# lifuguan/GGRt_official

Measured on AMD Instinct MI355X. Metric: Gaussian raster fwd+bwd Mpix/s @1M Gaussians 1080p, higher is better.
Workload: dtype f32; 1 GPU; C3: 1000000 Gaussians, 1920x1080, SH deg 3, profile A, fwd+bwd incl. camera gradient, 1 frame per GPU; parallelism=frames x1

## Files before the change

ggrt_official_amd/csrc/api.hip:

```cpp
#include "../../include/ggr_raster.h"
#include "ggr_common.h"
#include "blend_feat.h"
#include "blend_contrib.h"
#include "blend_pick.h"
#include "blend_dist.h"
#include <algorithm>
#include <mutex>
#include <vector>

#include <stdarg.h>
#include <stdio.h>
#include <stdlib.h>
#include <string.h>
#include <time.h>

namespace {

thread_local char g_err[512] = "";
const char kSpinFault[] = "depth sort: a look-back spin hit its bound (GPU preempted or halted?); frame not rendered";
const char kRangeFault[] = "depth sort: a sort key beyond 30 bits reached the sort (keys must come from preprocess_fwd); frame not rendered";

int fail(int code, const char* fmt, ...) {
    va_list ap;
    va_start(ap, fmt);
// ... 665 lines not shown
        uint32_t two[2] = {0u, 0u};
        HIP_TRY(hipMemcpyAsync(two, g.counters, 8, hipMemcpyDeviceToHost, s));
        HIP_TRY(hipStreamSynchronize(s));
        if (two[1] & 2u) return fail(GGR_E_HIP, "%s", kSpinFault);
        if (two[1] & 4u) return fail(GGR_E_LIMIT, "%s", kRangeFault);
    }
    if (bucket_slow && out->depth_sort_used == GGR_DEPTH_SORT_GLOBAL) out->depth_sort_used = GGR_DEPTH_SORT_GLOBAL_SLOW;
    tm.finish();
    if (out->stage_ms && side) {
        float ms = 0.f;
        if (hipEventElapsedTime(&ms, side->t0, side->t1) == hipSuccess) out->stage_ms[GGR_FWD_COLOUR] += ms;
        else (void)hipGetLastError();
    }
    return GGR_OK;
}

int backward_impl(const GgrSettings* st, const ViewSet& vs, const GgrBackwardIn* in, GgrBackwardOut* out, void* stream,
                  const float* dL_dalpha) {
    if (!out) return fail(GGR_E_INVALID, "null gradient output struct");
    const int NV = vs.V;
    if (st->num_points == 0) {
        hipStream_t s0 = (hipStream_t)stream;
        if (out->dL_dviewmatrix) HIP_TRY(hipMemsetAsync(out->dL_dviewmatrix, 0, 64 * (size_t)NV, s0));
        if (out->dL_dprojmatrix) HIP_TRY(hipMemsetAsync(out->dL_dprojmatrix, 0, 64 * (size_t)NV, s0));
        if (out->dL_dcampos) HIP_TRY(hipMemsetAsync(out->dL_dcampos, 0, 12 * (size_t)NV, s0));
        return GGR_OK;
    }
    if (!out->dL_dmeans3D || !out->dL_dmeans2D || !out->dL_dopacities || !out->dL_dcov3D)
        return fail(GGR_E_INVALID, "null gradient output");
    if (!in->geom_buffer || !in->image_buffer || !in->scratch || !in->dL_dout_color)
        return fail(GGR_E_INVALID, "null saved buffer / scratch / upstream gradient");
    const bool has_cp = in->fwd.colors_precomp != nullptr;
    if (has_cp ? !out->dL_dcolors_precomp : !out->dL_dshs) return fail(GGR_E_INVALID, "null colour gradient output");
    const bool has_sr = in->fwd.scales != nullptr;
    if (has_sr && (!out->dL_dscales || !out->dL_drotations)) return fail(GGR_E_INVALID, "null scale/rotation gradient output");
    if (in->fwd.aux_precomp && in->dL_dout_depth && !out->dL_daux) return fail(GGR_E_INVALID, "null dL_daux output");
    const int npose = (out->dL_dviewmatrix != nullptr) + (out->dL_dprojmatrix != nullptr) + (out->dL_dcampos != nullptr);
    if (npose != 0 && npose != 3) return fail(GGR_E_INVALID, "camera gradients: give all three outputs or none");
    hipStream_t s = (hipStream_t)stream;
    const int P = st->num_points, W = st->image_width, H = st->image_height;
    const bool dbg = st->debug != 0;
    if (in->num_rendered != 0 && !in->binning_buffer) return fail(GGR_E_INVALID, "null binning buffer");

    GeomLayout g = ggr_carve_geom((void*)in->geom_buffer, (size_t)P * NV, ggr_sort_segments((size_t)NV));
    ImageLayout im = ggr_carve_image((void*)in->image_buffer, W, H, NV);
    const uint32_t* point_list = (const uint32_t*)in->binning_buffer;
    BwdScratch sc = ggr_carve_bwd(in->scratch, (size_t)P, (size_t)NV);

    StageTimer tm(s, out->stage_ms, GGR_BWD_STAGES);
    if (!in->scratch_zeroed)
        HIP_TRY(hipMemsetAsync(in->scratch, 0, sc.bytes, s));
    tm.mark(GGR_BWD_CLEAR);

    if (in->num_rendered != 0) {
        ggr::launch_blend_bwd(W, H, im.ranges, point_list, g.splat, g.colour, vs.bg, im.final_T, im.n_contrib,
                              in->dL_dout_color, in->dL_dout_depth, dL_dalpha, sc.grad2d, im.tile_top, im.ckpt,
                              im.ckpt_slots, im.bwd_segments, NV, s);
        KCHECK(dbg, s, "blend_bwd");
    }
    tm.mark(GGR_BWD_BLEND);
    const float* cov = in->fwd.cov3D_precomp ? in->fwd.cov3D_precomp : g.cov3D;
    ggr::launch_preprocess_bwd(P, st->sh_degree, st->sh_stride, in->fwd.means3D, in->fwd.shs, g.sh_jac, has_cp ? 1 : 0,
                               in->fwd.scales, in->fwd.rotations, st->scale_modifier, cov, vs, W, H, in->radii, g.clamped,
                               sc.grad2d, in->dL_dout_depth ? 1 : 0, out->dL_dmeans3D, out->dL_dmeans2D,
                               out->dL_dopacities, out->dL_dshs, out->dL_dcolors_precomp, out->dL_dcov3D,
                               out->dL_dscales, out->dL_drotations, in->fwd.aux_precomp ? out->dL_daux : nullptr,
                               npose ? sc.pose_acc : nullptr, out->dL_dviewmatrix, out->dL_dprojmatrix,
                               out->dL_dcampos, input_form(st, &in->fwd, vs.sets, out->dL_dshs), in->fwd.cov3D_precomp ? 1 : 0,
                               in->fwd.opacities, g.counters + GGR_CTR_ANTIALIAS , s);
    KCHECK(dbg, s, "preprocess_bwd");
    tm.mark(GGR_BWD_PREPROCESS);
    return GGR_OK;
}

}

extern "C" {

int ggr_forward_ext(const GgrSettings* st, const GgrForwardOptions* opt, const GgrForwardExtra* ex, const GgrForwardIn* in,
                    GgrForwardOut* out, GgrAllocFn alloc, void* alloc_ctx, void* stream) {
    g_err[0] = 0;
    int aa = 0;
    int rc = validate_options(opt, &aa);
    if (rc) return rc;
    if ((rc = validate_extra(ex, "GgrForwardExtra")) != 0) return rc;
    rc = validate(st, in);
    if (rc) return rc;
    return forward_impl(st, single_view(st, in), in, out, alloc, alloc_ctx, stream, aa, ex ? ex->out_alpha : nullptr);
}

int ggr_forward_opt(const GgrSettings* st, const GgrForwardOptions* opt, const GgrForwardIn* in, GgrForwardOut* out,
                    GgrAllocFn alloc, void* alloc_ctx, void* stream) {
    return ggr_forward_ext(st, opt, nullptr, in, out, alloc, alloc_ctx, stream);
}

int ggr_forward(const GgrSettings* st, const GgrForwardIn* in, GgrForwardOut* out, GgrAllocFn alloc,
                void* alloc_ctx, void* stream) {
    return ggr_forward_ext(st, nullptr, nullptr, in, out, alloc, alloc_ctx, stream);
}

int ggr_backward_ext(const GgrSettings* st, const GgrBackwardExtra* ex, const GgrBackwardIn* in, GgrBackwardOut* out,
                     void* stream) {
    g_err[0] = 0;
    int rc = validate_extra(ex, "GgrBackwardExtra");
    if (rc) return rc;
    if (!in) return fail(GGR_E_INVALID, "null inputs");
    rc = validate(st, &in->fwd);
    if (rc) return rc;
    return backward_impl(st, single_view(st, &in->fwd), in, out, stream, ex ? ex->dL_dout_alpha : nullptr);
}
// ... 430 lines not shown
```

ggrt_official_amd/csrc/blend_bwd.hip:

```cpp
#include "blend_common.h"

namespace ggr {

#define BATCH GGR_BATCH
#define RB 8

__device__ unsigned long long g_bwd_counters[4];
void blend_bwd_counters(unsigned long long* out, int reset) {
    (void)hipMemcpyFromSymbol(out, HIP_SYMBOL(g_bwd_counters), sizeof(g_bwd_counters));
    if (reset) { const unsigned long long z[4] = {0, 0, 0, 0}; (void)hipMemcpyToSymbol(HIP_SYMBOL(g_bwd_counters), z, sizeof z); }
}

template <int CTRL>
__device__ __forceinline__ float dpp_mov(float v) {
    return __int_as_float(__builtin_amdgcn_update_dpp(__float_as_int(v), __float_as_int(v), CTRL, 0xf, 0xf, true));
}

__device__ __forceinline__ float transpose_rows8(float (&v)[RB], int lane) {
    float w4[4];
    const bool h32 = (lane & 32) != 0;
#pragma unroll
    for (int i = 0; i < 4; i++) {
        const float keep = h32 ? v[i + 4] : v[i], send = h32 ? v[i] : v[i + 4];
        w4[i] = keep + __int_as_float(__builtin_amdgcn_ds_bpermute((lane ^ 32) << 2, __float_as_int(send)));
    }
    float w2[2];
#pragma unroll
    for (int i = 0; i < 2; i++) {
        const auto r = __builtin_amdgcn_permlane16_swap(__float_as_uint(w4[i]), __float_as_uint(w4[i + 2]), false, false);
        w2[i] = __uint_as_float(r[0]) + __uint_as_float(r[1]);
    }
    const bool hi = (lane & 8) != 0;
    const float keep = hi ? w2[1] : w2[0];
    const float send = hi ? w2[0] : w2[1];
    return keep + dpp_mov<0x128>(send);
}

__device__ __forceinline__ float sum_cols8(float s) {
    s += dpp_mov<0xB1>(s);
    s += dpp_mov<0x4E>(s);
    s += dpp_mov<0x141>(s);
    asm volatile("" : "+v"(s));
    return s;
}

__device__ __forceinline__ float transpose_cols8(const float (&o)[8], int lane) {
    const bool up = (lane & 4) != 0;
    const bool e0 = (((lane ^ (lane >> 2)) & 1) != 0), e1 = ((((lane >> 1) ^ (lane >> 2)) & 1) != 0);
    float k1[4], k2[2];
#pragma unroll
    for (int i = 0; i < 4; i++) {
        const float keep = e0 ? o[2 * i + 1] : o[2 * i], send = e0 ? o[2 * i] : o[2 * i + 1];
        k1[i] = keep + dpp_mov<0xB1>(send);
    }
#pragma unroll
    for (int j = 0; j < 2; j++) {
        const float keep = e1 ? k1[2 * j + 1] : k1[2 * j], send = e1 ? k1[2 * j] : k1[2 * j + 1];
        k2[j] = keep + dpp_mov<0x4E>(send);
    }
    const float keep = up ? k2[1] : k2[0], send = up ? k2[0] : k2[1];
    return keep + dpp_mov<0x141>(send);
}

template <bool HAS_DEPTH, bool HAS_ALPHA>
__global__ void __launch_bounds__(256)
blend_bwd_kernel(int W, int H, int grid_x, const uint2* __restrict__ ranges,
                 const uint32_t* __restrict__ point_list, const float4* __restrict__ splat,
                 const float4* __restrict__ colour,
                 const float* __restrict__ bg, const float* __restrict__ final_T,
                 const uint32_t* __restrict__ n_contrib, const float* __restrict__ dL_dpix,
                 const float* __restrict__ dL_ddepth, const float* __restrict__ dL_dalpha, float* __restrict__ grad2d,
                 const uint32_t* __restrict__ tile_top, const float* __restrict__ ckpt, int ckpt_slots,
                 int segments, int views) {
    __shared__ StagedSplat stage[BATCH];
    __shared__ __attribute__((aligned(16))) uint16_t surv[4][BATCH];
    __shared__ uint32_t wave_top[4];

    const int tid = threadIdx.x, lane = tid & 63, wave = tid >> 6;
    const int tiles1 = grid_x * ((H + GGR_TILE - 1) / GGR_TILE), ntiles = tiles1 * views;
    const int seg = segments > 1 ? (int)blockIdx.x / xcd_grid(ntiles) : 0;
    const int vtile = xcd_tile((int)blockIdx.x - seg * xcd_grid(ntiles), ntiles, true);
    if (vtile < 0) return;
    const int view = vtile / tiles1, tile = vtile - view * tiles1;
    const int tile_x = tile % grid_x, tile_y = tile / grid_x;
    const int qx0 = tile_x * GGR_TILE + (wave & 1) * 8, qy0 = tile_y * GGR_TILE + (wave >> 1) * 8;
    const int px = qx0 + (lane & 7), py = qy0 + (lane >> 3);
    const bool inside = px < W && py < H;
    const float pixx = (float)px, pixy = (float)py;
    const float rx0 = (float)qx0, ry0 = (float)qy0;
    const float qcx = rx0 + 3.5f, qcy = ry0 + 3.5f;
    const float pxc = (float)(lane & 7) - 3.5f, pyc = (float)(lane >> 3) - 3.5f;
    const float rx1 = (float)min(qx0 + 7, W - 1), ry1 = (float)min(qy0 + 7, H - 1);

    const uint2 range = ranges[vtile];
    const int top = (int)min(tile_top[vtile], range.y - range.x);
    int seg_lo = 0, seg_hi = top, stride = 0;
    if (segments > 1) {
        stride = ckpt_stride((int)(range.y - range.x), ckpt_slots, ntiles);
        seg_lo = seg * stride;
        seg_hi = min(top, seg_lo + stride);
    }
    if (seg_lo >= seg_hi) return;
    const size_t hw = (size_t)H * W;
    const size_t pid = inside ? (size_t)py * W + px : 0;
    {
        const size_t vo = (size_t)view * hw;
        final_T += vo; n_contrib += vo; dL_dpix += 3 * vo; bg += 3 * view;
        if (HAS_DEPTH) dL_ddepth += vo;
        if (HAS_ALPHA) dL_dalpha += vo;
        if (ckpt) ckpt += (size_t)ckpt_slots * GGR_CKPT_FLOATS * vo;
    }

    const float T_final = inside ? final_T[pid] : 0.f;
    uint32_t last = inside ? n_contrib[pid] : 0u;
    float dp0 = 0.f, dp1 = 0.f, dp2 = 0.f, dpz = 0.f, dpa = 0.f;
    if (inside) {
        dp0 = dL_dpix[pid]; dp1 = dL_dpix[hw + pid]; dp2 = dL_dpix[2 * hw + pid];
        if (HAS_DEPTH) dpz = dL_ddepth[pid];
        if (HAS_ALPHA) dpa = dL_dalpha[pid];
    }
    if (dp0 == 0.f && dp1 == 0.f && dp2 == 0.f && dpz == 0.f && (!HAS_ALPHA || dpa == 0.f)) last = 0u;
    const float bg_dot = bg[0] * dp0 + bg[1] * dp1 + bg[2] * dp2;
    const float ddelx_dx = 0.5f * (float)W, ddely_dy = 0.5f * (float)H;

    uint32_t wl = last;
#pragma unroll
    for (int off = 32; off > 0; off >>= 1) wl = max(wl, (uint32_t)__shfl_xor((int)wl, off));
    if (lane == 0) wave_top[wave] = wl;
    __syncthreads();
    seg_hi = min(seg_hi, (int)max(max(wave_top[0], wave_top[1]), max(wave_top[2], wave_top[3])));
    if (seg_lo >= seg_hi) return;

    float T = T_final;
    float R = T_final * (HAS_ALPHA ? bg_dot - dpa : bg_dot);
    float amax = GGR_ALPHA_MAX, amin = GGR_ALPHA_MIN;
    __asm__ volatile("" : "+s"(amax), "+s"(amin));

    if (stride > 0 && seg_hi == seg_lo + stride && last > (uint32_t)seg_hi) {
        const float* ck = ckpt + (size_t)(seg_hi / stride) * GGR_CKPT_FLOATS * hw + pid;
        const float* fin = ckpt + pid;
        T = ck[0];
        R += (fin[hw] - ck[hw]) * dp0 + (fin[2 * hw] - ck[2 * hw]) * dp1 + (fin[3 * hw] - ck[3 * hw]) * dp2;
        if (HAS_DEPTH) R += (fin[4 * hw] - ck[4 * hw]) * dpz;
    }

    const int vi = lane & 7;
    const int vix = vi < 4 ? vi : 11 - vi;
    const int my_slot = lane >> 3;
// ... 98 lines not shown
                float val = 0.f;
                uint32_t gid = 0u;
                {
                    const int e = max(my_e, 0);
                    const float4 a = stage[e].a;
                    const float4 b = stage[e].b;
                    gid = __float_as_uint(stage[e].c.w);
                    const float op = b.y;
                    const float ox = a.x - qcx, oy = a.y - qcy;
                    const float Mx = pxc * Cm, Mxx = pxc * Mx, Mxy = pxc * Cy;
                    const float Sx = ox * Cm - Mx, Sy = oy * Cm - Cy;
                    o[3] = -op * GGR_INV_KQ * (a.z * Sx + 0.5f * a.w * Sy) * ddelx_dx;
                    o[4] = -op * GGR_INV_KQ * (b.x * Sy + 0.5f * a.w * Sx) * ddely_dy;
                    o[5] = -0.5f * op * (ox * (Sx - Mx) + Mxx);
                    o[6] = -0.5f * op * (ox * Sy - oy * Mx + Mxy);
                    o[7] = -0.5f * op * (oy * (Sy - Cy) + Cyy);
                    val = transpose_cols8(o, lane);
                }
                if (my_e < 0) val = 0.f;
                static_assert(GGR_G2D_Z == GGR_G2D_OPACITY + 1, "opacity and depth are committed as one pair");
                constexpr int NPAIR = HAS_DEPTH ? 2 : 1;
                const float pair_own = my_e < 0 ? 0.f : ((HAS_DEPTH && vi == 1) ? t_z : S0);
                const float pair_nb = dpp_mov<0x128>(pair_own);
                const uint32_t gid_nb = __float_as_uint(dpp_mov<0x128>(__uint_as_float(gid)));
                const bool odd = (my_slot & 1) != 0;
                float* const rec_own = grad2d + GGR_G2D_STRIDE * (size_t)gid;
                float* const rec_nb = grad2d + GGR_G2D_STRIDE * (size_t)gid_nb;
                const bool help = vi < NPAIR && pair_nb != 0.f;
                {
                    float* const p = odd ? rec_nb + GGR_G2D_OPACITY + vi : rec_own + vix;
                    const float v = odd ? pair_nb : val;
                    if (odd ? help : v != 0.f) atomicAdd(p, v);
                }
                {
                    float* const p = odd ? rec_own + vix : rec_nb + GGR_G2D_OPACITY + vi;
                    const float v = odd ? val : pair_nb;
                    if (odd ? v != 0.f : help) atomicAdd(p, v);
                }
            }
        }
    }
#ifdef GGR_DEV_COUNTERS
    if (lane == 0) {
        atomicAdd(&g_bwd_counters[0], dc_slots); atomicAdd(&g_bwd_counters[1], dc_dead);
        atomicAdd(&g_bwd_counters[2], dc_pairs); atomicAdd(&g_bwd_counters[3], dc_batches);
    }
#endif
}

void launch_blend_bwd(int W, int H, const uint2* ranges, const uint32_t* point_list, const float4* splat,
                      const float4* colour,
                      const float* bg, const float* final_T, const uint32_t* n_contrib,
                      const float* dL_dpix, const float* dL_ddepth, const float* dL_dalpha, float* grad2d,
                      const uint32_t* tile_top, const float* ckpt, int ckpt_slots, int segments, int views, hipStream_t s) {
    const int gx = (W + GGR_TILE - 1) / GGR_TILE, gy = (H + GGR_TILE - 1) / GGR_TILE;
    if (gx * gy * views == 0) return;
    const int nt = gx * gy * views;
    segments = (ckpt && ckpt_slots >= 2) ? ckpt_slots : 1;
#define GGR_LAUNCH_BBWD(DEPTH_, ALPHA_)                                                                                      \
    hipLaunchKernelGGL(HIP_KERNEL_NAME(blend_bwd_kernel<DEPTH_, ALPHA_>), dim3(xcd_grid(nt) * segments), dim3(256), 0, s, W, H, gx,  \
                       ranges, point_list, splat, colour, bg, final_T, n_contrib, dL_dpix, dL_ddepth, dL_dalpha, grad2d,       \
                       tile_top, ckpt, ckpt_slots, segments, views)
    if (dL_dalpha) {
        if (dL_ddepth) GGR_LAUNCH_BBWD(true, true);
        else GGR_LAUNCH_BBWD(false, true);
    } else {
        if (dL_ddepth) GGR_LAUNCH_BBWD(true, false);
        else GGR_LAUNCH_BBWD(false, false);
    }
#undef GGR_LAUNCH_BBWD
}

}
```

ggrt_official_amd/csrc/ggr_common.h:

```cpp
#pragma once
#include <hip/hip_runtime.h>
#include <stdint.h>
#include <stddef.h>

#define GGR_TILE 16
#define GGR_TILE_PIX 256
#define GGR_NEAR_CULL 0.2f
#define GGR_DILATION 0.3f
#define GGR_FRUSTUM_CLAMP 1.3f
#define GGR_ALPHA_MIN (1.0f / 255.0f)
#define GGR_ALPHA_MAX 0.99f
#define GGR_T_MIN 0.0001f
#define GGR_AA_MIN_RATIO 0.000025f

#define GGR_SORT_THREADS 512
#define GGR_SORT_ITEMS 8
#define GGR_SORT_TILE (GGR_SORT_THREADS * GGR_SORT_ITEMS)
#define GGR_KEY_BASE 0x3E4CCCCDu
#define GGR_KEY_MAX 0x3FFFFFFFu
#define GGR_SORT_PASSES 3
#define GGR_SORT_MAX_BITS 10
#define GGR_SORT_MAX_BINS (1 << GGR_SORT_MAX_BITS)
#define GGR_PRE_THREADS 256

// ... 265 lines not shown
};
TileListPlan plan_tile_lists(size_t P, size_t T);
void launch_tile_list_count(const TileListPlan& pl, size_t P, size_t T, int grid_x, const uint32_t* order,
                            const uint2* rect, void* work, uint2* ranges, uint32_t* total_out, uint32_t capacity,
                            hipStream_t s, bool rects_gathered = false ,
                            uint32_t* host_total = nullptr ,
                            hipEvent_t after_scan = nullptr ,
                            const uint32_t* sort_fault = nullptr ,
                            bool id_order = false ,
                            uint32_t list_limit = 0xFFFFFFFFu );
const uint32_t* radix_sort_fault_word(const uint32_t* hist);
void tile_list_gather_targets(const TileListPlan& pl, void* work, size_t T, uint2** rect_sorted,
                              uint32_t** zero_area, uint32_t* zero_words);
void launch_tile_list_ranges(const TileListPlan& pl, size_t T, void* work, uint2* ranges, hipStream_t s);
void launch_tile_list_scatter(const TileListPlan& pl, size_t P, size_t T, int grid_x, const uint32_t* order,
                              const uint2* rect, const void* work, uint32_t* point_list, uint32_t capacity,
                              hipStream_t s, const uint32_t* keys = nullptr ,
                              uint2* pair_list = nullptr );

struct TileSortExtras {
    const uint2* gather_src;
    uint2* gather_dst;
    uint32_t* zero_area;
    uint32_t zero_words;
    uint32_t* fault_word;
};
void launch_bucket_sort_big(uint32_t segments, const uint2* ranges, uint32_t* point_list, const uint2* pair_list, uint32_t min_len,
                            hipStream_t s, TileSortExtras ex);
void launch_tile_depth_sort(size_t T, const uint2* ranges, uint32_t* point_list, const uint2* pair_list, uint32_t min_len,
                            uint32_t max_len, hipStream_t s, int copy_longer ,
                            uint32_t* lsd_entries = nullptr ,
                            const TileSortExtras* extras = nullptr);


void launch_blend_fwd(int W, int H, const uint2* ranges, const uint32_t* point_list, const float4* splat,
                      const float4* colour,
                      const float* bg, float* out_color, float* final_T, uint32_t* n_contrib,
                      float* out_depth, float* out_alpha , float* ckpt ,
                      int ckpt_slots, uint32_t* tile_top, int views,
                      int scissored ,
                      void* zero_area , size_t zero_bytes ,
                      hipStream_t s);

void blend_fwd_counters(unsigned long long* out4, int reset);
void blend_bwd_counters(unsigned long long* out4, int reset);

void launch_blend_bwd(int W, int H, const uint2* ranges, const uint32_t* point_list, const float4* splat,
                      const float4* colour,
                      const float* bg, const float* final_T, const uint32_t* n_contrib,
                      const float* dL_dpix, const float* dL_ddepth ,
                      const float* dL_dalpha ,
                      float* grad2d ,
                      const uint32_t* tile_top, const float* ckpt , int ckpt_slots, int segments, int views,
                      hipStream_t s);

void launch_preprocess_bwd(int P, int D, int M, const float* means3D, const float* shs ,
                           const float4* sh_jac ,
                           int has_colors_precomp, const float* scales, const float* rotations,
                           float scale_modifier, const float* cov3D, ViewSet vs, int W, int H, const int32_t* radii,
                           const uint32_t* clamped,
                           const float* grad2d, int has_dz, float* dL_dmeans3D, float* dL_dmeans2D,
                           float* dL_dopacity, float* dL_dsh,
                           float* dL_dcolors_precomp, float* dL_dcov3D, float* dL_dscales,
                           float* dL_drotations, float* dL_daux, float* pose_acc ,
                           float* dL_dview, float* dL_dproj, float* dL_dcampos, InputForm inf,
                           int cov_is_input ,
                           const float* opacities ,
                           const uint32_t* mode_word , hipStream_t s);

void launch_mark_visible(int P, const float* means3D, const float* viewmatrix, uint8_t* present,
                         hipStream_t s);

void launch_camera_setup(int n, const float* extrinsics, const float* intrinsics, const float* near, const float* far,
                         int scale_invariant, float* view, float* full, float* campos, float* tanfov, float* scale,
                         hipStream_t s);

void launch_copy_f4(const void* src, void* dst, size_t bytes, int blocks , hipStream_t s);
void launch_spin(unsigned long long ticks, uint32_t* started , hipStream_t s);
void launch_noop(hipStream_t s);

void launch_unpack_geom(GeomLayout g, int P, float* depth, float* xy, float* conic_opacity, float* rgb,
                        int32_t* tiles_touched, uint8_t* clamped, hipStream_t s);

}
```

ggrt_official_amd/csrc/preprocess_bwd.hip:

```cpp
#include "ggr_common.h"
#include "sh_stage.h"
#include "sh_terms.h"
#include <algorithm>

namespace ggr {

template <int CTRL, int ROW_MASK = 0xf>
__device__ __forceinline__ float dpp_take(float v) {
    return __int_as_float(__builtin_amdgcn_update_dpp(0, __float_as_int(v), CTRL, ROW_MASK, 0xf, false));
}
__device__ __forceinline__ float wave_sum_lane63(float v) {
    v += dpp_take<0x111>(v);
    v += dpp_take<0x112>(v);
    v += dpp_take<0x114>(v);
    v += dpp_take<0x118>(v);
    v += dpp_take<0x142, 0xa>(v);
    v += dpp_take<0x143, 0xc>(v);
    return v;
}

#define GGR_SH_MAXK 25

__device__ __forceinline__ void sh_basis25(int deg, float x, float y, float z, float* B) {
    B[0] = SH_C0;
    if (deg > 0) {
        B[1] = -SH_C1 * y; B[2] = SH_C1 * z; B[3] = -SH_C1 * x;
        if (deg > 1) {
            const float xx = x * x, yy = y * y, zz = z * z, xy = x * y, yz = y * z, xz = x * z;
            B[4] = bSH_C2[0] * xy; B[5] = bSH_C2[1] * yz; B[6] = bSH_C2[2] * (2.f * zz - xx - yy);
            B[7] = bSH_C2[3] * xz; B[8] = bSH_C2[4] * (xx - yy);
            if (deg > 2) {
                B[9] = bSH_C3[0] * y * (3.f * xx - yy);
                B[10] = bSH_C3[1] * xy * z;
                B[11] = bSH_C3[2] * y * (4.f * zz - xx - yy);
                B[12] = bSH_C3[3] * z * (2.f * zz - 3.f * xx - 3.f * yy);
                B[13] = bSH_C3[4] * x * (4.f * zz - xx - yy);
                B[14] = bSH_C3[5] * z * (xx - yy);
                B[15] = bSH_C3[6] * x * (xx - 3.f * yy);
                if (deg > 3) {
                    B[16] = bSH_C4[0] * xy * (xx - yy);
                    B[17] = bSH_C4[1] * yz * (3.f * xx - yy);
                    B[18] = bSH_C4[2] * xy * (7.f * zz - 1.f);
                    B[19] = bSH_C4[3] * yz * (7.f * zz - 3.f);
                    B[20] = bSH_C4[4] * (zz * (35.f * zz - 30.f) + 3.f);
                    B[21] = bSH_C4[5] * xz * (7.f * zz - 3.f);
                    B[22] = bSH_C4[6] * (xx - yy) * (7.f * zz - 1.f);
                    B[23] = bSH_C4[7] * xz * (xx - 3.f * yy);
                    B[24] = bSH_C4[8] * (xx * (xx - 3.f * yy) - yy * (3.f * xx - yy));
                }
            }
        }
    }
}

template <bool POSE, bool MULTI, int KC, bool CM>
__global__ void __launch_bounds__(256)
preprocess_bwd_kernel(int P, int D, int M, const float* __restrict__ means3D, const float* __restrict__ shs,
                      const float4* __restrict__ sh_jac, size_t jac_plane, int has_colors_precomp, const float* __restrict__ scales,
                      const float* __restrict__ rotations, float scale_modifier,
                      const float* __restrict__ cov3D, ViewSet vs, int W, int H,
                      const int32_t* __restrict__ radii,
                      const uint32_t* __restrict__ clamped, const float* __restrict__ grad2d, int has_dz,
                      float* __restrict__ dL_dmeans3D, float* __restrict__ dL_dmeans2D,
                      float* __restrict__ dL_dopacity, float* __restrict__ dL_dsh, float* __restrict__ dL_dcolors_precomp,
                      float* __restrict__ dL_dcov3D, float* __restrict__ dL_dscales,
                      float* __restrict__ dL_drotations, float* __restrict__ dL_daux,
                      float* __restrict__ pose_acc, InputForm inf, int cov_is_input,
                      const float* __restrict__ opacities, const uint32_t* __restrict__ mode_word) {
    extern __shared__ __attribute__((aligned(16))) float sh_lds[];
    const int i = blockIdx.x * blockDim.x + threadIdx.x;
    const bool aa = mode_word[0] != 0u;
    const bool in_range = i < P;
    const int NV = MULTI ? vs.vps : 1;
    {
// ... 236 lines not shown
                for (int ii = 0; ii < 3; ii++)
#pragma unroll
                    for (int j = 0; j < 3; j++) Mx[3 * ii + j] = R[3 * ii + j] * sc[j];
                const float dS[9] = {dcv[0], 0.5f * dcv[1], 0.5f * dcv[2], 0.5f * dcv[1], dcv[3], 0.5f * dcv[4],
                                     0.5f * dcv[2], 0.5f * dcv[4], dcv[5]};
                float dR[9];
#pragma unroll
                for (int j = 0; j < 3; j++) {
                    float acc = 0.f;
#pragma unroll
                    for (int ii = 0; ii < 3; ii++) {
                        float dMij = 0.f;
#pragma unroll
                        for (int k = 0; k < 3; k++) dMij += dS[3 * ii + k] * Mx[3 * k + j];
                        dMij *= 2.f;
                        acc += dMij * R[3 * ii + j];
                        dR[3 * ii + j] = dMij * sc[j];
                    }
                    dsc[j] += acc * sm;
                }
                drot[0] += 2.f * (z * (dR[3] - dR[1]) + y * (dR[2] - dR[6]) + x * (dR[7] - dR[5]));
                drot[1] += 2.f * (y * (dR[1] + dR[3]) + z * (dR[2] + dR[6]) + r * (dR[7] - dR[5])) - 4.f * x * (dR[4] + dR[8]);
                drot[2] += 2.f * (x * (dR[1] + dR[3]) + r * (dR[2] - dR[6]) + z * (dR[5] + dR[7])) - 4.f * y * (dR[0] + dR[8]);
                drot[3] += 2.f * (r * (dR[3] - dR[1]) + x * (dR[2] + dR[6]) + y * (dR[5] + dR[7])) - 4.f * z * (dR[0] + dR[4]);
            }
        }
        if (POSE) {
            __shared__ float wred[4][40];
            const int lane = threadIdx.x & 63, wave = threadIdx.x >> 6;
#pragma unroll
            for (int k = 0; k < 16; k++) {
                const float sv = wave_sum_lane63(dV[k]);
                const float sp = wave_sum_lane63(dPM[k]);
                if (lane == 63) { wred[wave][k] = sv; wred[wave][16 + k] = sp; }
            }
            if (lane == 63) { wred[wave][32] = 0.f; wred[wave][33] = 0.f; wred[wave][34] = 0.f; }
            __syncthreads();
            if (threadIdx.x < 35)
                pose_acc[((size_t)v * gridDim.x + blockIdx.x) * 64 + threadIdx.x] =
                    wred[0][threadIdx.x] + wred[1][threadIdx.x] + wred[2][threadIdx.x] + wred[3][threadIdx.x];
            __syncthreads();
        }
    }

    if (use_sh && KC > 0) {
        constexpr int KCN = KC > 0 ? KC : 1, DEG = KC == 16 ? 3 : 4;
        const float4 c0 = recs[(GGR_G2D_STRIDE / 4) * il];
        const bool live = in_range && radii[il] > 0;
        const uint32_t cl = clamped[il];
        const float4 j0 = ggr_ld_f4(reinterpret_cast<const float*>(sh_jac + il)),
                     j1 = ggr_ld_f4(reinterpret_cast<const float*>(sh_jac + jac_plane + il)),
                     j2 = ggr_ld_f4(reinterpret_cast<const float*>(sh_jac + 2 * jac_plane + il));
        float dc[3] = {live && !(cl & 1u) ? c0.x : 0.f, live && !(cl & 2u) ? c0.y : 0.f, live && !(cl & 4u) ? c0.z : 0.f};
        const float in_s = vs.input_scale ? vs.input_scale[0] : 1.0f;
        const float vx = live ? in_s * m0 - vs.campos[0] : 0.f, vy = live ? in_s * m1 - vs.campos[1] : 0.f,
                    vz = live ? in_s * m2 - vs.campos[2] : 1.f;
        const float len = sqrtf(vx * vx + vy * vy + vz * vz);
        float x = vx / len, y = vy / len, z = vz / len;
        const float ddx = live ? j0.x * dc[0] + j1.x * dc[1] + j2.x * dc[2] : 0.f;
        const float ddy = live ? j0.y * dc[0] + j1.y * dc[1] + j2.y * dc[2] : 0.f;
        const float ddz = live ? j0.z * dc[0] + j1.z * dc[1] + j2.z * dc[2] : 0.f;
        constexpr bool cm = CM;
        float dcam[3] = {0.f, 0.f, 0.f};
        if (live) {
            const float sum2 = vx * vx + vy * vy + vz * vz;
            const float inv32 = 1.0f / sqrtf(sum2 * sum2 * sum2);
            const float gx_ = ((sum2 - vx * vx) * ddx - vy * vx * ddy - vz * vx * ddz) * inv32;
            const float gy_ = (-vx * vy * ddx + (sum2 - vy * vy) * ddy - vz * vy * ddz) * inv32;
            const float gz_ = (-vx * vz * ddx - vy * vz * ddy + (sum2 - vz * vz) * ddz) * inv32;
            dmean[0] += in_s * gx_; dmean[1] += in_s * gy_; dmean[2] += in_s * gz_;
            if (POSE) { dcam[0] = -gx_; dcam[1] = -gy_; dcam[2] = -gz_; }
        }
        if (POSE) {
            __shared__ float cred3[4][4];
            const int lane = threadIdx.x & 63, wave = threadIdx.x >> 6;
#pragma unroll
            for (int k = 0; k < 3; k++) {
                const float scm = wave_sum_lane63(dcam[k]);
                if (lane == 63) cred3[wave][k] = scm;
            }
            __syncthreads();
            if (threadIdx.x >= 32 && threadIdx.x < 35) {
                const int k = threadIdx.x - 32;
                pose_acc[(size_t)blockIdx.x * 64 + threadIdx.x] += cred3[0][k] + cred3[1][k] + cred3[2][k] + cred3[3][k];
            }
        }
        const int rowlen = (int)sh_row;
        const int pk = cm ? 1 : 3, pc = cm ? M : 1;
#pragma unroll 1
        for (int R = 0; R < 3; R++) {
            const int r0 = 84 * R, r1 = R == 2 ? 256 : r0 + 84;
            __syncthreads();
            if ((int)threadIdx.x >= r0 && (int)threadIdx.x < r1 && in_range) {
                float* rowp = sh_lds + ((int)threadIdx.x - r0) * rowlen;
#define SH_ROW(k, Bk, bx, by, bz) { const float b_ = (Bk); rowp[(k) * pk] = b_ * dc[0]; rowp[(k) * pk + pc] = b_ * dc[1]; rowp[(k) * pk + 2 * pc] = b_ * dc[2]; }
                GGR_SH_TERMS(SH_ROW, DEG, )
#undef SH_ROW
                for (int k = KCN; k < M; k++) { rowp[k * pk] = 0.f; rowp[k * pk + pc] = 0.f; rowp[k * pk + 2 * pc] = 0.f; }
            }
            __syncthreads();
            const int nrow = min(r1, nG) - r0;
            if (nrow > 0) {
                const int total = nrow * rowlen, n4 = total >> 2;
                float* dst = dL_dsh + (g0 + r0) * sh_row;
                for (int j = threadIdx.x; j < n4; j += 256)
                    ggr_st_f4(dst + 4 * (size_t)j, reinterpret_cast<const float4*>(sh_lds)[j]);
                for (int j = (n4 << 2) + threadIdx.x; j < total; j += 256) ggr_st(dst + j, sh_lds[j]);
            }
        }
    } else if (use_sh) {
        float4 q0 = recs[(GGR_G2D_STRIDE / 4) * il];
        int qrad = radii[il];
        uint32_t qcl = clamped[il];
#pragma clang loop unroll(disable)
        for (int v = 0; v < NV; v++) {
            __asm__ volatile("" ::: "memory");
            const size_t o = (size_t)v * P + il;
            const float4 r0 = q0;
            const bool live = in_range && qrad > 0;
            const uint32_t cl = qcl;
            if (MULTI && v + 1 < NV) { q0 = recs[(GGR_G2D_STRIDE / 4) * (o + P)]; qrad = radii[o + P]; qcl = clamped[o + P]; }
            float dcam[3] = {0.f, 0.f, 0.f};
            if (live) {
            float dc0 = r0.x, dc1 = r0.y, dc2 = r0.z;
            const float in_s = vs.input_scale ? vs.input_scale[v] : 1.0f;
            const float p0 = in_s * m0, p1 = in_s * m1, p2 = in_s * m2;
            const float* campos = vs.campos + 3 * v;
            float dmv[3] = {0.f, 0.f, 0.f};
            {
            if (cl & 1u) dc0 = 0.f;
            if (cl & 2u) dc1 = 0.f;
            if (cl & 4u) dc2 = 0.f;
            const float vx = p0 - campos[0], vy = p1 - campos[1], vz = p2 - campos[2];
            const float len = sqrtf(vx * vx + vy * vy + vz * vz);
            const float x = vx / len, y = vy / len, z = vz / len;
            float* dsh1 = sh_lds + threadIdx.x * sh_stride;
            const float4 j0 = ggr_ld_f4(reinterpret_cast<const float*>(sh_jac + o)),
                         j1 = ggr_ld_f4(reinterpret_cast<const float*>(sh_jac + jac_plane + o)),
                         j2 = ggr_ld_f4(reinterpret_cast<const float*>(sh_jac + 2 * jac_plane + o));
            const float ddx = j0.x * dc0 + j1.x * dc1 + j2.x * dc2;
            const float ddy = j0.y * dc0 + j1.y * dc1 + j2.y * dc2;
            const float ddz = j0.z * dc0 + j1.z * dc1 + j2.z * dc2;
#define SH_TERM(k, Bk, bx, by, bz)                                                                     \
{                                                                                                  \
    const int o0 = (k) * sh_ks, o1 = o0 + sh_cs, o2 = o1 + sh_cs;                                  \
    dsh1[o0] = (Bk) * dc0; dsh1[o1] = (Bk) * dc1; dsh1[o2] = (Bk) * dc2;                           \
}
            if (!MULTI) GGR_SH_TERMS(SH_TERM, deg, )
#undef SH_TERM
            const float sum2 = vx * vx + vy * vy + vz * vz;
            const float inv32 = 1.0f / sqrtf(sum2 * sum2 * sum2);
            const float gx_ = ((sum2 - vx * vx) * ddx - vy * vx * ddy - vz * vx * ddz) * inv32;
            const float gy_ = (-vx * vy * ddx + (sum2 - vy * vy) * ddy - vz * vy * ddz) * inv32;
            const float gz_ = (-vx * vz * ddx - vy * vz * ddy + (sum2 - vz * vz) * ddz) * inv32;
            dmv[0] += gx_; dmv[1] += gy_; dmv[2] += gz_;
            if (POSE) { dcam[0] -= gx_; dcam[1] -= gy_; dcam[2] -= gz_; }

            }
            dmean[0] += in_s * dmv[0]; dmean[1] += in_s * dmv[1]; dmean[2] += in_s * dmv[2];
            }
            if (POSE) {
                __shared__ float cred[4][4];
                const int lane = threadIdx.x & 63, wave = threadIdx.x >> 6;
#pragma unroll
                for (int k = 0; k < 3; k++) {
                    const float scm = wave_sum_lane63(dcam[k]);
                    if (lane == 63) cred[wave][k] = scm;
                }
                __syncthreads();
                if (threadIdx.x >= 32 && threadIdx.x < 35) {
                    const int k = threadIdx.x - 32;
                    pose_acc[((size_t)v * gridDim.x + blockIdx.x) * 64 + threadIdx.x] += cred[0][k] + cred[1][k] + cred[2][k] + cred[3][k];
                }
                __syncthreads();
            }
        }
        float* dsh = sh_lds + threadIdx.x * sh_stride;
        if (!MULTI) {
            if (in_range && !(radii[il] > 0)) {
                for (int k = 0; k < (sh_compact ? sh_rowf : sh_flat ? (int)sh_row : copy_row); k++) dsh[k] = 0.f;
            } else if (in_range && !sh_compact) {
                if (inf.sh_channel_major) {
                    for (int c = 0; c < 3; c++)
                        for (int k = K; k < M; k++) dsh[c * M + k] = 0.f;
                } else if (sh_flat) {
                    for (int k = sh_rowf; k < (int)sh_row; k++) dsh[k] = 0.f;
                }
            }
        }
        __syncthreads();
        if (sh_compact) {
            write_sh_rows_compact(dL_dsh, sh_lds, g0, nG, M, sh_rowf / 3, sh_stride, inf.sh_channel_major != 0);
        } else if (sh_flat) {
            const size_t total = (size_t)nG * sh_row;
            float* dst = dL_dsh + g0 * sh_row;
            const int n4 = (int)(total >> 2);
            for (int j = threadIdx.x; j < n4; j += blockDim.x)
                ggr_st_f4(dst + 4 * (size_t)j, reinterpret_cast<const float4*>(sh_lds)[j]);
            for (int j = (n4 << 2) + threadIdx.x; j < (int)total; j += blockDim.x) ggr_st(dst + j, sh_lds[j]);
        } else if ((sh_row & 3) == 0 && (sh_rowf & 3) == 0) {
            const int q_row = (int)(sh_row >> 2), q_used = copy_row >> 2;
            for (int j = threadIdx.x; j < nG * q_row; j += blockDim.x) {
                const int g = j / q_row, q = j - g * q_row;
                float4 v4 = make_float4(0.f, 0.f, 0.f, 0.f);
                if (q < q_used) {
                    const float* d = sh_lds + g * sh_stride + 4 * q;
                    v4 = make_float4(d[0], d[1], d[2], d[3]);
                }
                ggr_st_f4(dL_dsh + (g0 + g) * sh_row + 4 * q, v4);
            }
        } else {
            const int wv = threadIdx.x >> 6, ln = threadIdx.x & 63, nw = blockDim.x >> 6;
#pragma unroll 8
            for (int g = wv; g < nG; g += nw)
                for (int k = ln; k < (int)sh_row; k += 64)
                    ggr_st(dL_dsh + (g0 + g) * sh_row + k, k < copy_row ? sh_lds[g * sh_stride + k] : 0.f);
        }
    }
    if (in_range) {
        ggr_st(dL_dopacity + i, dop);
        ggr_st(dL_dmeans3D + 3 * i, dmean[0]); ggr_st(dL_dmeans3D + 3 * i + 1, dmean[1]); ggr_st(dL_dmeans3D + 3 * i + 2, dmean[2]);
        if (has_colors_precomp) { ggr_st(dL_dcolors_precomp + 3 * i, dcp[0]); ggr_st(dL_dcolors_precomp + 3 * i + 1, dcp[1]); ggr_st(dL_dcolors_precomp + 3 * i + 2, dcp[2]); }
        if (scales && dL_dscales) {
            dL_dscales[3 * i] = dsc[0]; dL_dscales[3 * i + 1] = dsc[1]; dL_dscales[3 * i + 2] = dsc[2];
            dL_drotations[4 * i] = drot[0]; dL_drotations[4 * i + 1] = drot[1]; dL_drotations[4 * i + 2] = drot[2];
            dL_drotations[4 * i + 3] = drot[3];
        }
        if (cov_is_input && inf.cov_stride == 9) {
            float* d9 = dL_dcov3D + 9 * (size_t)i;
            d9[0] = dcov[0]; d9[1] = dcov[1]; d9[2] = dcov[2];
            d9[3] = 0.f;     d9[4] = dcov[3]; d9[5] = dcov[4];
            d9[6] = 0.f;     d9[7] = 0.f;     d9[8] = dcov[5];
        } else {
#pragma unroll
            for (int k = 0; k < 6; k++) ggr_st(dL_dcov3D + 6 * (size_t)i + k, dcov[k]);
        }
    }
}

#ifndef GGR_SHV_WAVES
#define GGR_SHV_WAVES 1
#endif
template <int KMAX, bool POSE>
__global__ void __launch_bounds__(256, GGR_SHV_WAVES)
preprocess_bwd_sh_views_kernel(int P, int M, int deg, const float* __restrict__ means3D, const float* __restrict__ shs,
                               const float4* __restrict__ sh_jac, size_t jac_plane, ViewSet vs, const int32_t* __restrict__ radii, const uint32_t* __restrict__ clamped,
                               const float* __restrict__ grad2d, float* __restrict__ dL_dmeans3D,
                               float* __restrict__ dL_dsh, float* __restrict__ pose_acc, InputForm inf) {
    extern __shared__ __attribute__((aligned(16))) float sh_lds[];
    const int i = blockIdx.x * blockDim.x + threadIdx.x;
    const bool in_range = i < P;
    const size_t il = (size_t)min(i, P - 1);
    {
        const int set = (int)blockIdx.y, v0 = set * vs.vps;
        const size_t in_off = (size_t)set * (size_t)P, st_off = (size_t)v0 * (size_t)P;
        means3D += 3 * in_off; shs += in_off * (size_t)M * 3;
        dL_dmeans3D += 3 * in_off; dL_dsh += in_off * (size_t)M * 3;
        radii += st_off; clamped += st_off; grad2d += GGR_G2D_STRIDE * st_off; sh_jac += st_off;
        if (POSE) pose_acc += (size_t)v0 * gridDim.x * 64;
        vs.campos += 3 * v0;
        if (vs.input_scale) vs.input_scale += v0;
    }
    const float m0 = means3D[3 * il], m1 = means3D[3 * il + 1], m2 = means3D[3 * il + 2];
    const int K = (deg + 1) * (deg + 1);
    const size_t g0 = (size_t)blockIdx.x * blockDim.x;
    const int nG = (int)min((size_t)blockDim.x, (size_t)P - g0);
    const size_t sh_row = (size_t)M * 3;
    const int sh_rowf = 3 * K;
    const bool sh_flat = (sh_row & 1) != 0 && inf.sh_aligned != 0;
// ... 193 lines not shown
```

ggrt_official_amd/csrc/sh_stage.h:

```cpp
#pragma once
#include <hip/hip_runtime.h>
#include <stdint.h>

namespace ggr {

__device__ __forceinline__ void stage_sh_rows(float* __restrict__ sh_lds, const float* __restrict__ shs, size_t g0,
                                              int nG, size_t row, int copy_row, int stride, bool flat) {
    const int tid = threadIdx.x;
    if (flat) {
        const size_t total = (size_t)nG * row;
        const float* src = shs + g0 * row;
        const int n4 = (int)(total >> 2);
        constexpr int U = 19;
        for (int j0 = 0; j0 < n4; j0 += U * 256) {
            float4 v[U];
#pragma unroll
            for (int it = 0; it < U; it++) v[it] = ggr_ld_f4(src + 4 * (size_t)min(j0 + it * 256 + tid, n4 - 1));
#pragma unroll
            for (int it = 0; it < U; it++) {
                const int j = j0 + it * 256 + tid;
                if (j < n4) reinterpret_cast<float4*>(sh_lds)[j] = v[it];
            }
        }
        for (int j = (n4 << 2) + tid; j < (int)total; j += 256) sh_lds[j] = ggr_ld(src + j);
// ... 7 lines not shown
            for (int it = 0; it < 12; it++) {
                const int j = min(j0 + it * 256 + tid, total4 - 1);
                gg[it] = j / q_per;
                qq[it] = j - gg[it] * q_per;
                v[it] = ggr_ld_f4(shs + (g0 + gg[it]) * row + 4 * qq[it]);
            }
#pragma unroll
            for (int it = 0; it < 12; it++) {
                if (j0 + it * 256 + tid < total4) {
                    float* d = sh_lds + gg[it] * stride + 4 * qq[it];
                    d[0] = v[it].x; d[1] = v[it].y; d[2] = v[it].z; d[3] = v[it].w;
                }
            }
        }
    } else {
        const int wv = tid >> 6, ln = tid & 63;
#pragma unroll 8
        for (int g = wv; g < nG; g += 4)
            for (int k = ln; k < copy_row; k += 64) sh_lds[g * stride + k] = ggr_ld(shs + (g0 + g) * row + k);
    }
}

__device__ __forceinline__ void stage_sh_rows_compact(float* __restrict__ sh_lds, const float* __restrict__ shs,
                                                      size_t g0, int nG, int M, int K, int stride, bool channel_major) {
    const int tid = threadIdx.x, wv = tid >> 6, ln = tid & 63;
    const int row = 3 * M;
    int col[2] = {ln, ln + 64}, dst[2];
#pragma unroll
    for (int h = 0; h < 2; h++) {
        if (col[h] >= row) dst[h] = -1;
        else if (channel_major) { const int c = col[h] / M, k = col[h] - c * M; dst[h] = k < K ? c * K + k : -1; }
        else dst[h] = col[h] < 3 * K ? col[h] : -1;
    }
    const int c0 = min(col[0], row - 1), c1 = min(col[1], row - 1);
    for (int gb = wv * 8; gb < nG; gb += 32) {
        float v[16];
#pragma unroll
        for (int r = 0; r < 8; r++) {
            const size_t g = g0 + (size_t)min(gb + r, nG - 1);
            v[2 * r] = ggr_ld(shs + g * row + c0);
            v[2 * r + 1] = ggr_ld(shs + g * row + c1);
        }
#pragma unroll
        for (int r = 0; r < 8; r++) {
            if (gb + r < nG) {
                if (dst[0] >= 0) sh_lds[(gb + r) * stride + dst[0]] = v[2 * r];
                if (dst[1] >= 0) sh_lds[(gb + r) * stride + dst[1]] = v[2 * r + 1];
            }
        }
    }
}

__device__ __forceinline__ void write_sh_rows_compact(float* __restrict__ dL_dsh, const float* __restrict__ sh_lds,
                                                      size_t g0, int nG, int M, int K, int stride, bool channel_major) {
    const int tid = threadIdx.x, wv = tid >> 6, ln = tid & 63;
    const int row = 3 * M;
#pragma unroll
    for (int h = 0; h < 2; h++) {
        const int col = ln + 64 * h;
        if (col >= row) continue;
        int dst;
        if (channel_major) { const int c = col / M, k = col - c * M; dst = k < K ? c * K + k : -1; }
        else dst = col < 3 * K ? col : -1;
#pragma unroll 8
        for (int g = wv; g < nG; g += 4)
            ggr_st(dL_dsh + (g0 + g) * row + col, dst >= 0 ? sh_lds[g * stride + dst] : 0.f);
    }
}

template <int KC>
struct ShThirds {
    static constexpr int STRIDE = KC | 1, RPI = 256 / KC, ITS = (256 + RPI - 1) / RPI;
    const float* src;
    int g, k, last;
    uint32_t row;
    int step;
    __device__ __forceinline__ void init(const float* block_rows, int nG, int row_floats, int third_step) {
        src = block_rows; row = (uint32_t)row_floats; step = third_step; last = nG - 1;
        g = (int)threadIdx.x / KC; k = (int)threadIdx.x - g * KC;
    }
    __device__ __forceinline__ void load(float (&v)[ITS], int J) const {
        const float* s = src + J * step;
#pragma unroll
        for (int it = 0; it < ITS; it++) v[it] = s[(uint32_t)min(g + it * RPI, last) * row + (uint32_t)k];
    }
    __device__ __forceinline__ void store(float* lds, const float (&v)[ITS]) const {
#pragma unroll
        for (int it = 0; it < ITS; it++)
            if (g < RPI && g + it * RPI < 256) lds[(g + it * RPI) * STRIDE + k] = v[it];
    }
};

}
```

Before: 2656 Mpix/s.

## Pre-zero SH gradients inside blend backward and skip dead-row SH stores

The SH gradient output is now zeroed up front, either by a grid-stride float4 fill inside the blend backward kernel or by a memset when that path cannot be used. Preprocess backward then writes only SH rows whose Gaussian is live and has a nonzero colour gradient, tracked with a per-wave ballot bitmask in shared memory. The aim is to cut write traffic for culled Gaussians and hide the zero fill inside a compute-heavy kernel. In exchange, every blend block pays for extra stores, and correctness now depends on the pre-zeroing having covered every skipped row.

```diff
diff --git a/ggrt_official_amd/csrc/api.hip b/ggrt_official_amd/csrc/api.hip
--- a/ggrt_official_amd/csrc/api.hip
+++ b/ggrt_official_amd/csrc/api.hip
@@ -741,10 +741,19 @@
         HIP_TRY(hipMemsetAsync(in->scratch, 0, sc.bytes, s));
     tm.mark(GGR_BWD_CLEAR);
 
+    float* sh_fill = (!has_cp && vs.vps == 1) ? out->dL_dshs : nullptr;
+    const size_t sh_fill_floats = (size_t)vs.sets * (size_t)P * (size_t)st->sh_stride * 3;
+    const bool fill_in_blend = sh_fill && in->num_rendered != 0 && ((uintptr_t)sh_fill & 15) == 0;
+    if (sh_fill && !fill_in_blend) {
+        HIP_TRY(hipMemsetAsync(sh_fill, 0, sh_fill_floats * sizeof(float), s));
+    } else if (sh_fill && (sh_fill_floats & 3)) {
+        HIP_TRY(hipMemsetAsync(sh_fill + (sh_fill_floats & ~(size_t)3), 0, (sh_fill_floats & 3) * sizeof(float), s));
+    }
     if (in->num_rendered != 0) {
         ggr::launch_blend_bwd(W, H, im.ranges, point_list, g.splat, g.colour, vs.bg, im.final_T, im.n_contrib,
                               in->dL_dout_color, in->dL_dout_depth, dL_dalpha, sc.grad2d, im.tile_top, im.ckpt,
-                              im.ckpt_slots, im.bwd_segments, NV, s);
+                              im.ckpt_slots, im.bwd_segments, NV, fill_in_blend ? sh_fill : nullptr,
+                              fill_in_blend ? sh_fill_floats >> 2 : 0, s);
         KCHECK(dbg, s, "blend_bwd");
     }
     tm.mark(GGR_BWD_BLEND);
diff --git a/ggrt_official_amd/csrc/blend_bwd.hip b/ggrt_official_amd/csrc/blend_bwd.hip
--- a/ggrt_official_amd/csrc/blend_bwd.hip
+++ b/ggrt_official_amd/csrc/blend_bwd.hip
@@ -71,7 +71,7 @@
                  const uint32_t* __restrict__ n_contrib, const float* __restrict__ dL_dpix,
                  const float* __restrict__ dL_ddepth, const float* __restrict__ dL_dalpha, float* __restrict__ grad2d,
                  const uint32_t* __restrict__ tile_top, const float* __restrict__ ckpt, int ckpt_slots,
-                 int segments, int views) {
+                 int segments, int views, float* __restrict__ zero_fill, size_t zero_fill_n4) {
     __shared__ StagedSplat stage[BATCH];
     __shared__ __attribute__((aligned(16))) uint16_t surv[4][BATCH];
     __shared__ uint32_t wave_top[4];
@@ -80,6 +80,13 @@
     const int tiles1 = grid_x * ((H + GGR_TILE - 1) / GGR_TILE), ntiles = tiles1 * views;
     const int seg = segments > 1 ? (int)blockIdx.x / xcd_grid(ntiles) : 0;
     const int vtile = xcd_tile((int)blockIdx.x - seg * xcd_grid(ntiles), ntiles, true);
+    const uint2 range = ranges[max(vtile, 0)];
+    const uint32_t top_word = tile_top[max(vtile, 0)];
+    if (zero_fill) {
+        const float4 z4 = make_float4(0.f, 0.f, 0.f, 0.f);
+        for (size_t j = (size_t)blockIdx.x * 256 + tid; j < zero_fill_n4; j += (size_t)gridDim.x * 256)
+            ggr_st_f4(zero_fill + 4 * j, z4);
+    }
     if (vtile < 0) return;
     const int view = vtile / tiles1, tile = vtile - view * tiles1;
     const int tile_x = tile % grid_x, tile_y = tile / grid_x;
@@ -92,8 +99,7 @@
     const float pxc = (float)(lane & 7) - 3.5f, pyc = (float)(lane >> 3) - 3.5f;
     const float rx1 = (float)min(qx0 + 7, W - 1), ry1 = (float)min(qy0 + 7, H - 1);
 
-    const uint2 range = ranges[vtile];
-    const int top = (int)min(tile_top[vtile], range.y - range.x);
+    const int top = (int)min(top_word, range.y - range.x);
     int seg_lo = 0, seg_hi = top, stride = 0;
     if (segments > 1) {
         stride = ckpt_stride((int)(range.y - range.x), ckpt_slots, ntiles);
@@ -298,7 +304,8 @@
                       const float4* colour,
                       const float* bg, const float* final_T, const uint32_t* n_contrib,
                       const float* dL_dpix, const float* dL_ddepth, const float* dL_dalpha, float* grad2d,
-                      const uint32_t* tile_top, const float* ckpt, int ckpt_slots, int segments, int views, hipStream_t s) {
+                      const uint32_t* tile_top, const float* ckpt, int ckpt_slots, int segments, int views,
+                      float* zero_fill, size_t zero_fill_n4, hipStream_t s) {
     const int gx = (W + GGR_TILE - 1) / GGR_TILE, gy = (H + GGR_TILE - 1) / GGR_TILE;
     if (gx * gy * views == 0) return;
     const int nt = gx * gy * views;
@@ -306,7 +313,7 @@
 #define GGR_LAUNCH_BBWD(DEPTH_, ALPHA_)                                                                                      \
     hipLaunchKernelGGL(HIP_KERNEL_NAME(blend_bwd_kernel<DEPTH_, ALPHA_>), dim3(xcd_grid(nt) * segments), dim3(256), 0, s, W, H, gx,  \
                        ranges, point_list, splat, colour, bg, final_T, n_contrib, dL_dpix, dL_ddepth, dL_dalpha, grad2d,       \
-                       tile_top, ckpt, ckpt_slots, segments, views)
+                       tile_top, ckpt, ckpt_slots, segments, views, zero_fill, zero_fill_n4)
     if (dL_dalpha) {
         if (dL_ddepth) GGR_LAUNCH_BBWD(true, true);
         else GGR_LAUNCH_BBWD(false, true);
diff --git a/ggrt_official_amd/csrc/ggr_common.h b/ggrt_official_amd/csrc/ggr_common.h
--- a/ggrt_official_amd/csrc/ggr_common.h
+++ b/ggrt_official_amd/csrc/ggr_common.h
@@ -341,7 +341,8 @@
                       const float* dL_dalpha ,
                       float* grad2d ,
                       const uint32_t* tile_top, const float* ckpt , int ckpt_slots, int segments, int views,
-                      hipStream_t s);
+                      float* zero_fill ,
+                      size_t zero_fill_n4 , hipStream_t s);
 
 void launch_preprocess_bwd(int P, int D, int M, const float* means3D, const float* shs ,
                            const float4* sh_jac ,
diff --git a/ggrt_official_amd/csrc/preprocess_bwd.hip b/ggrt_official_amd/csrc/preprocess_bwd.hip
--- a/ggrt_official_amd/csrc/preprocess_bwd.hip
+++ b/ggrt_official_amd/csrc/preprocess_bwd.hip
@@ -20,6 +20,11 @@
 }
 
 #define GGR_SH_MAXK 25
+
+__device__ __forceinline__ bool sh_row_live(const unsigned long long* live_rows, int g) {
+    return ((live_rows[g >> 6] >> (g & 63)) & 1ull) != 0ull;
+}
+__device__ __forceinline__ int sh_row_of(int f, float inv) { return (int)(((float)f + 0.5f) * inv); }
 
 __device__ __forceinline__ void sh_basis25(int deg, float x, float y, float z, float* B) {
     B[0] = SH_C0;
@@ -362,6 +367,11 @@
                      j1 = ggr_ld_f4(reinterpret_cast<const float*>(sh_jac + jac_plane + il)),
                      j2 = ggr_ld_f4(reinterpret_cast<const float*>(sh_jac + 2 * jac_plane + il));
         float dc[3] = {live && !(cl & 1u) ? c0.x : 0.f, live && !(cl & 2u) ? c0.y : 0.f, live && !(cl & 4u) ? c0.z : 0.f};
+        __shared__ unsigned long long live_rows[4];
+        {
+            const unsigned long long lm = __ballot(live && (c0.x != 0.f || c0.y != 0.f || c0.z != 0.f));
+            if ((threadIdx.x & 63) == 0) live_rows[threadIdx.x >> 6] = lm;
+        }
         const float in_s = vs.input_scale ? vs.input_scale[0] : 1.0f;
         const float vx = live ? in_s * m0 - vs.campos[0] : 0.f, vy = live ? in_s * m1 - vs.campos[1] : 0.f,
                     vz = live ? in_s * m2 - vs.campos[2] : 1.f;
@@ -396,6 +406,7 @@
             }
         }
         const int rowlen = (int)sh_row;
+        const float inv_rowlen = 1.0f / (float)rowlen;
         const int pk = cm ? 1 : 3, pc = cm ? M : 1;
 #pragma unroll 1
         for (int R = 0; R < 3; R++) {
@@ -414,14 +425,22 @@
                 const int total = nrow * rowlen, n4 = total >> 2;
                 float* dst = dL_dsh + (g0 + r0) * sh_row;
                 for (int j = threadIdx.x; j < n4; j += 256)
-                    ggr_st_f4(dst + 4 * (size_t)j, reinterpret_cast<const float4*>(sh_lds)[j]);
-                for (int j = (n4 << 2) + threadIdx.x; j < total; j += 256) ggr_st(dst + j, sh_lds[j]);
+                    if (sh_row_live(live_rows, r0 + sh_row_of(4 * j, inv_rowlen)) ||
+                        sh_row_live(live_rows, r0 + sh_row_of(4 * j + 3, inv_rowlen)))
+                        ggr_st_f4(dst + 4 * (size_t)j, reinterpret_cast<const float4*>(sh_lds)[j]);
+                for (int j = (n4 << 2) + threadIdx.x; j < total; j += 256)
+                    if (sh_row_live(live_rows, r0 + sh_row_of(j, inv_rowlen))) ggr_st(dst + j, sh_lds[j]);
             }
         }
     } else if (use_sh) {
         float4 q0 = recs[(GGR_G2D_STRIDE / 4) * il];
         int qrad = radii[il];
         uint32_t qcl = clamped[il];
+        __shared__ unsigned long long live_rows[4];
+        if (!MULTI) {
+            const unsigned long long lm = __ballot(in_range && qrad > 0 && (q0.x != 0.f || q0.y != 0.f || q0.z != 0.f));
+            if ((threadIdx.x & 63) == 0) live_rows[threadIdx.x >> 6] = lm;
+        }
 #pragma clang loop unroll(disable)
         for (int v = 0; v < NV; v++) {
             __asm__ volatile("" ::: "memory");
@@ -488,7 +507,8 @@
         float* dsh = sh_lds + threadIdx.x * sh_stride;
         if (!MULTI) {
             if (in_range && !(radii[il] > 0)) {
-                for (int k = 0; k < (sh_compact ? sh_rowf : sh_flat ? (int)sh_row : copy_row); k++) dsh[k] = 0.f;
+                if (sh_flat && !sh_compact)
+                    for (int k = 0; k < (int)sh_row; k++) dsh[k] = 0.f;
             } else if (in_range && !sh_compact) {
                 if (inf.sh_channel_major) {
                     for (int c = 0; c < 3; c++)
@@ -500,18 +520,22 @@
         }
         __syncthreads();
         if (sh_compact) {
-            write_sh_rows_compact(dL_dsh, sh_lds, g0, nG, M, sh_rowf / 3, sh_stride, inf.sh_channel_major != 0);
+            write_sh_rows_compact(dL_dsh, sh_lds, live_rows, g0, nG, M, sh_rowf / 3, sh_stride, inf.sh_channel_major != 0);
         } else if (sh_flat) {
             const size_t total = (size_t)nG * sh_row;
             float* dst = dL_dsh + g0 * sh_row;
             const int n4 = (int)(total >> 2);
+            const float inv_row = 1.0f / (float)sh_row;
             for (int j = threadIdx.x; j < n4; j += blockDim.x)
-                ggr_st_f4(dst + 4 * (size_t)j, reinterpret_cast<const float4*>(sh_lds)[j]);
-            for (int j = (n4 << 2) + threadIdx.x; j < (int)total; j += blockDim.x) ggr_st(dst + j, sh_lds[j]);
+                if (sh_row_live(live_rows, sh_row_of(4 * j, inv_row)) || sh_row_live(live_rows, sh_row_of(4 * j + 3, inv_row)))
+                    ggr_st_f4(dst + 4 * (size_t)j, reinterpret_cast<const float4*>(sh_lds)[j]);
+            for (int j = (n4 << 2) + threadIdx.x; j < (int)total; j += blockDim.x)
+                if (sh_row_live(live_rows, sh_row_of(j, inv_row))) ggr_st(dst + j, sh_lds[j]);
         } else if ((sh_row & 3) == 0 && (sh_rowf & 3) == 0) {
             const int q_row = (int)(sh_row >> 2), q_used = copy_row >> 2;
             for (int j = threadIdx.x; j < nG * q_row; j += blockDim.x) {
                 const int g = j / q_row, q = j - g * q_row;
+                if (!sh_row_live(live_rows, g)) continue;
                 float4 v4 = make_float4(0.f, 0.f, 0.f, 0.f);
                 if (q < q_used) {
                     const float* d = sh_lds + g * sh_stride + 4 * q;
@@ -522,9 +546,11 @@
         } else {
             const int wv = threadIdx.x >> 6, ln = threadIdx.x & 63, nw = blockDim.x >> 6;
 #pragma unroll 8
-            for (int g = wv; g < nG; g += nw)
+            for (int g = wv; g < nG; g += nw) {
+                if (!sh_row_live(live_rows, g)) continue;
                 for (int k = ln; k < (int)sh_row; k += 64)
                     ggr_st(dL_dsh + (g0 + g) * sh_row + k, k < copy_row ? sh_lds[g * sh_stride + k] : 0.f);
+            }
         }
     }
     if (in_range) {
diff --git a/ggrt_official_amd/csrc/sh_stage.h b/ggrt_official_amd/csrc/sh_stage.h
--- a/ggrt_official_amd/csrc/sh_stage.h
+++ b/ggrt_official_amd/csrc/sh_stage.h
@@ -83,7 +83,7 @@
 }
 
 __device__ __forceinline__ void write_sh_rows_compact(float* __restrict__ dL_dsh, const float* __restrict__ sh_lds,
-                                                      size_t g0, int nG, int M, int K, int stride, bool channel_major) {
+                                                      const unsigned long long* live_rows, size_t g0, int nG, int M, int K, int stride, bool channel_major) {
     const int tid = threadIdx.x, wv = tid >> 6, ln = tid & 63;
     const int row = 3 * M;
 #pragma unroll
@@ -95,7 +95,8 @@
         else dst = col < 3 * K ? col : -1;
 #pragma unroll 8
         for (int g = wv; g < nG; g += 4)
-            ggr_st(dL_dsh + (g0 + g) * row + col, dst >= 0 ? sh_lds[g * stride + dst] : 0.f);
+            if ((live_rows[g >> 6] >> (g & 63)) & 1ull)
+                ggr_st(dL_dsh + (g0 + g) * row + col, dst >= 0 ? sh_lds[g * stride + dst] : 0.f);
     }
 }
 
```

Measured after the change: 2654 Mpix/s. About the same (-0.1%).
